# cornell-zhang/HiSparse

Hardware: AMD Instinct MI355X
Metric: SpMV GBPS (8 B per non-zero per SpMV, sw/benchmark.cpp:312-346) (higher is better)
Workload: dtype u32 (Q8.24 fixed point, u64 row sums)

## Files before the change

### hisparse_amd/csrc/spmv_device.h

```cpp
#ifndef HISPARSE_SPMV_DEVICE_H_
#define HISPARSE_SPMV_DEVICE_H_

#include <hip/hip_runtime.h>

#include <type_traits>

#include "stream_tiles.h"

namespace hisparse {
namespace dev {
namespace {

__device__ __forceinline__ uint32_t q8_24_mul(uint32_t a, uint32_t b) {
    const uint64_t wide = static_cast<uint64_t>(a) * b + 0x800000ull;
    uint32_t hi = static_cast<uint32_t>(wide >> 32);
    const uint32_t lo = static_cast<uint32_t>(wide);
    asm("" : "+v"(hi));
    const uint32_t r = __builtin_amdgcn_alignbit(hi, lo, 24);
    return (hi >> 24) ? 0xffffffffu : r;
}

typedef const __attribute__((address_space(4))) Unit* UnitTable;
typedef const __attribute__((address_space(4))) Block* BlockTable;

template <bool kFloat>
struct Rows;
template <>
struct Rows<false> {
    using acc_t = unsigned long long;
    using prod_t = unsigned long long;
    static __device__ __forceinline__ prod_t product(uint32_t mat, uint32_t vec) { return q8_24_mul(mat, vec); }
    static __device__ __forceinline__ void add(acc_t* ys, uint32_t row, prod_t p) { atomicAdd(ys + row, p); }
    static __device__ __forceinline__ uint32_t finish(acc_t s) { return s > 0xffffffffull ? 0xffffffffu : static_cast<uint32_t>(s); }
    using sum_t = unsigned long long;
    static __device__ __forceinline__ sum_t widen(prod_t p) { return p; }
    static __device__ __forceinline__ void add_sum(acc_t* ys, uint32_t row, sum_t v) { atomicAdd(ys + row, v); }
    using lane_t = unsigned long long;
    static __device__ __forceinline__ void add_lane(acc_t* ys, uint32_t row, lane_t v) { atomicAdd(ys + row, v); }
};
template <>
struct Rows<true> {
    using acc_t = double;
    using prod_t = float;
    static __device__ __forceinline__ prod_t product(uint32_t mat, uint32_t vec) { return __uint_as_float(mat) * __uint_as_float(vec); }
    static __device__ __forceinline__ void add(acc_t* ys, uint32_t row, prod_t p) { atomicAdd(ys + row, static_cast<double>(p)); }
    static __device__ __forceinline__ uint32_t finish(acc_t s) { return __float_as_uint(static_cast<float>(s)); }
    using sum_t = double;
    static __device__ __forceinline__ sum_t widen(prod_t p) { return static_cast<double>(p); }
    static __device__ __forceinline__ void add_sum(acc_t* ys, uint32_t row, sum_t v) { atomicAdd(ys + row, v); }
    using lane_t = float;
    static __device__ __forceinline__ void add_lane(acc_t* ys, uint32_t row, lane_t v) { atomicAdd(ys + row, static_cast<double>(v)); }
};

template <typename T>
__device__ __forceinline__ T wave_sum(T v) {
#pragma unroll
    for (int m = 32; m >= 1; m >>= 1) v += __shfl_xor(v, m, kWaveLanes);
    return v;
}

template <int kCtrl, int kRowMask>
__device__ __forceinline__ uint32_t dpp_from(uint32_t v) {
    return static_cast<uint32_t>(__builtin_amdgcn_update_dpp(0, static_cast<int>(v), kCtrl, kRowMask, 0xf, false));
}
template <int kCtrl, int kRowMask>
__device__ __forceinline__ unsigned long long dpp_from(unsigned long long v) {
    const uint32_t lo = dpp_from<kCtrl, kRowMask>(static_cast<uint32_t>(v)), hi = dpp_from<kCtrl, kRowMask>(static_cast<uint32_t>(v >> 32));
    return static_cast<unsigned long long>(hi) << 32 | lo;
}
template <int kCtrl, int kRowMask>
__device__ __forceinline__ double dpp_from(double v) {
    return __longlong_as_double(static_cast<long long>(dpp_from<kCtrl, kRowMask>(static_cast<unsigned long long>(__double_as_longlong(v)))));
}
template <typename T>
__device__ __forceinline__ T wave_inclusive_scan(T v);
template <typename T>
__device__ __forceinline__ T wave_total_in_lane63(T v) { return wave_inclusive_scan(v); }
template <typename T>
__device__ __forceinline__ T wave_inclusive_scan(T v) {
    v += dpp_from<0x111, 0xf>(v);
    v += dpp_from<0x112, 0xf>(v);
    v += dpp_from<0x114, 0xf>(v);
    v += dpp_from<0x118, 0xf>(v);
    v += dpp_from<0x142, 0xa>(v);
    v += dpp_from<0x143, 0xc>(v);
    return v;
}

template <int kCtrl, int kRowMask, typename T>
__device__ __forceinline__ void segmented_step(T& v, uint32_t row) {
    const uint32_t from_row = static_cast<uint32_t>(__builtin_amdgcn_update_dpp(-1, static_cast<int>(row), kCtrl, kRowMask, 0xf, false));
    const T arriving = dpp_from<kCtrl, kRowMask>(v);
    if (from_row == row) v += arriving;
}
template <typename T>
__device__ __forceinline__ T segmented_run_sums(T v, uint32_t row, bool& is_last) {
    segmented_step<0x111, 0xf>(v, row);
    segmented_step<0x112, 0xf>(v, row);
    segmented_step<0x114, 0xf>(v, row);
    segmented_step<0x118, 0xf>(v, row);
    segmented_step<0x142, 0xa>(v, row);
    segmented_step<0x143, 0xc>(v, row);
    const uint32_t next_row = static_cast<uint32_t>(__builtin_amdgcn_update_dpp(-1, static_cast<int>(row), 0x130, 0xf, 0xf, false));
    is_last = next_row != row;
    return v;
}


struct CarriedCombine {
    const uint32_t* partial = nullptr;
    uint32_t* y = nullptr;
    uint32_t num_rows = 0;
    uint32_t slices = 0;
};

// ... 48 lines not shown
```

### hisparse_amd/csrc/spmv_kernels.hip

```cpp
#include <hip/hip_runtime.h>

#include <cstdio>
#include <cstdlib>
#include <utility>
#include <vector>

#include "spmv_kernels.h"
#include "spmv_device.h"

namespace hisparse {
namespace dev {

namespace {

constexpr int kThreads = kWaveLanes * kWavesPerWorkgroup;
constexpr int kLightThreads = 256;
#ifndef HS_LIGHT_BATCH
#define HS_LIGHT_BATCH 4
#endif
constexpr int kLightBatch = HS_LIGHT_BATCH;
constexpr uint32_t kBufBytes = kSubTileCols * 4u;

template <int kIters, int kStride>
__device__ __forceinline__ void fill_x(uint32_t* dst, const uint32_t* __restrict__ x, uint32_t col0, uint32_t ncols, uint32_t t) {
// ... 20 lines not shown
}
template <int kFills>
__device__ __forceinline__ void dma_wait() {
    asm volatile("s_waitcnt vmcnt(%0)" ::"n"(kFills * kDmaPerFill) : "memory");
}

#ifndef HS_ROWBLOCK_STREAM_POLICY
#define HS_ROWBLOCK_STREAM_POLICY "nt"
#endif
#ifndef HS_ROWBLOCK_RESIDENT_POLICY
#define HS_ROWBLOCK_RESIDENT_POLICY "sc1"
#endif
#define HS_BY_POLICY(kRes, STATEMENT)                                 \
    do {                                                              \
        if constexpr (kRes) { STATEMENT(HS_ROWBLOCK_RESIDENT_POLICY); } \
        else { STATEMENT(HS_ROWBLOCK_STREAM_POLICY); }                \
    } while (0)
#define HS_RING_AGPRS "a0", "a1", "a2", "a3", "a4", "a5", "a6", "a7", "a8", "a9", "a10", "a11", "a12", "a13", "a14", "a15", "a16", "a17", \
                      "a18", "a19", "a20", "a21", "a22", "a23", "a24", "a25", "a26", "a27", "a28", "a29", "a30", "a31"
constexpr int kMaxDepth = 16;
constexpr int kOwner24Depth = 3;

constexpr int ring_format(int kRing) { return (kRing & 8) ? 4 : (kRing & 3); }
constexpr bool ring_is_delta(int kRing) { return ring_format(kRing) == 1 || ring_format(kRing) == 4; }
template <int kFmt, bool kRes>
struct RingT;
template <int kRing>
using Ring = RingT<ring_format(kRing), (kRing & 4) != 0>;
template <bool kRes>
struct RingT<0, kRes> {
    static constexpr uint32_t kLaneBytes = 8;
    template <int K>
    static __device__ __forceinline__ void issue(const uint8_t* base, uint32_t byte_off, uint32_t lane_off) {
#define HS_ISSUE(P) asm volatile("s_nop 4\n\tglobal_load_dwordx2 a[%0:%1], %2, %3 " P ::"n"(2 * K), "n"(2 * K + 1), "v"(byte_off + lane_off), "s"(base) : "memory", HS_RING_AGPRS)
        HS_BY_POLICY(kRes, HS_ISSUE);
#undef HS_ISSUE
    }
    template <int K, int kDepth>
    static __device__ __forceinline__ void take(uint32_t& value, uint32_t& where) {
        asm volatile("s_waitcnt vmcnt(%4)\n\tv_accvgpr_read_b32 %0, a[%2]\n\tv_accvgpr_read_b32 %1, a[%3]"
                     : "=v"(value), "=v"(where) : "n"(2 * K), "n"(2 * K + 1), "n"(kDepth - 1) : "memory");
    }
    template <int K, int kDepth>
    static __device__ __forceinline__ void take2(uint32_t& value0, uint32_t& where0, uint32_t& value1, uint32_t& where1) {
        asm volatile("s_waitcnt vmcnt(%8)\n\tv_accvgpr_read_b32 %0, a[%4]\n\tv_accvgpr_read_b32 %1, a[%5]\n\tv_accvgpr_read_b32 %2, a[%6]\n\t"
                     "v_accvgpr_read_b32 %3, a[%7]"
                     : "=v"(value0), "=v"(where0), "=v"(value1), "=v"(where1)
                     : "n"(2 * K), "n"(2 * K + 1), "n"(2 * K + 2), "n"(2 * K + 3), "n"(kDepth - 2) : "memory");
    }
};
template <bool kRes>
struct RingT<1, kRes> {
    static constexpr uint32_t kLaneBytes = 8;
    template <int K>
    static __device__ __forceinline__ void issue(const uint8_t* base, uint32_t byte_off, uint32_t lane_off) {
        static_assert(2 * K + 1 < kMaxDepth && K + kMaxDepth < 2 * kMaxDepth, "values in a0..a15, gap words in a16..a23: ring depth <= 8");
#define HS_ISSUE(P)                                                                                                                                         \
    asm volatile("s_nop 4\n\tglobal_load_dwordx2 a[%0:%1], %3, %5 " P "\n\tglobal_load_dword a[%2], %4, %5 offset:512 " P ::"n"(2 * K), "n"(2 * K + 1),     \
                 "n"(K + kMaxDepth), "v"(byte_off + lane_off), "v"(byte_off + lane_off / 2), "s"(base)                                                     \
                 : "memory", HS_RING_AGPRS)
        HS_BY_POLICY(kRes, HS_ISSUE);
#undef HS_ISSUE
    }
    template <int K, int kDepth>
    static __device__ __forceinline__ void take_record(uint32_t& value_a, uint32_t& value_b, uint32_t& gaps) {
        asm volatile("s_waitcnt vmcnt(%6)\n\tv_accvgpr_read_b32 %0, a[%3]\n\tv_accvgpr_read_b32 %1, a[%4]\n\tv_accvgpr_read_b32 %2, a[%5]"
                     : "=v"(value_a), "=v"(value_b), "=v"(gaps) : "n"(2 * K), "n"(2 * K + 1), "n"(K + kMaxDepth), "n"(2 * (kDepth - 1)) : "memory");
    }
};
template <bool kRes>
struct RingT<4, kRes> {
    static constexpr uint32_t kLaneBytes = 8;
    template <int K>
    static __device__ __forceinline__ void issue(const uint8_t* base, uint32_t byte_off, uint32_t lane_off) {
        static_assert(2 * K + 1 < kMaxDepth && K + kMaxDepth < 2 * kMaxDepth, "dwordx2 in a0..a15, gap B in a16..a23: ring depth <= 8");
#define HS_ISSUE(P)                                                                                                                                         \
    asm volatile("s_nop 4\n\tglobal_load_dwordx2 a[%0:%1], %3, %5 " P "\n\tglobal_load_ushort a[%2], %4, %5 offset:512 " P ::"n"(2 * K), "n"(2 * K + 1),    \
                 "n"(K + kMaxDepth), "v"(byte_off + lane_off), "v"(byte_off + lane_off / 4), "s"(base)                                                     \
                 : "memory", HS_RING_AGPRS)
        HS_BY_POLICY(kRes, HS_ISSUE);
#undef HS_ISSUE
    }
    template <int K, int kDepth>
    static __device__ __forceinline__ void take_record(uint32_t& field_a, uint32_t& field_b, uint32_t& gaps) {
        uint32_t lo, hi, gap_b;
        asm volatile("s_waitcnt vmcnt(%6)\n\tv_accvgpr_read_b32 %0, a[%3]\n\tv_accvgpr_read_b32 %1, a[%4]\n\tv_accvgpr_read_b32 %2, a[%5]"
                     : "=v"(lo), "=v"(hi), "=v"(gap_b) : "n"(2 * K), "n"(2 * K + 1), "n"(K + kMaxDepth), "n"(2 * (kDepth - 1)) : "memory");
        field_a = lo & 0xffffffu;
        field_b = __builtin_amdgcn_alignbit(hi, lo, 24) & 0xffffffu;
        gaps = (hi >> 16) | (gap_b << 16);
    }
};
template <bool kRes>
struct RingT<2, kRes> {
    static constexpr uint32_t kLaneBytes = 4;
    template <int K>
    static __device__ __forceinline__ void issue(const uint8_t* base, uint32_t byte_off, uint32_t lane_off) {
#define HS_ISSUE(P)                                                                                                                       \
    asm volatile("s_nop 4\n\tglobal_load_dword a[%0], %2, %4 " P "\n\tglobal_load_dword a[%1], %3, %4 offset:256 " P ::"n"(K),           \
                 "n"(K + kMaxDepth), "v"(byte_off + lane_off), "v"(byte_off + lane_off - lane_off / 4), "s"(base)                        \
                 : "memory", HS_RING_AGPRS)
        HS_BY_POLICY(kRes, HS_ISSUE);
#undef HS_ISSUE
    }
    template <int K, int kDepth>
    static __device__ __forceinline__ void take(uint32_t& value, uint32_t& where) {
        asm volatile("s_waitcnt vmcnt(%4)\n\tv_accvgpr_read_b32 %0, a[%2]\n\tv_accvgpr_read_b32 %1, a[%3]"
                     : "=v"(value), "=v"(where) : "n"(K), "n"(K + kMaxDepth), "n"(2 * (kDepth - 1)) : "memory");
        where &= 0xffffffu;
    }
    template <int K, int kDepth>
    static __device__ __forceinline__ void take2(uint32_t& value0, uint32_t& where0, uint32_t& value1, uint32_t& where1) {
        asm volatile("s_waitcnt vmcnt(%8)\n\tv_accvgpr_read_b32 %0, a[%4]\n\tv_accvgpr_read_b32 %1, a[%5]\n\tv_accvgpr_read_b32 %2, a[%6]\n\t"
                     "v_accvgpr_read_b32 %3, a[%7]"
                     : "=v"(value0), "=v"(where0), "=v"(value1), "=v"(where1)
                     : "n"(K), "n"(K + kMaxDepth), "n"(K + 1), "n"(K + 1 + kMaxDepth), "n"(2 * (kDepth - 2)) : "memory");
        where0 &= 0xffffffu;
        where1 &= 0xffffffu;
    }
};
template <bool kRes>
struct RingT<3, kRes> {
    template <int K>
    static __device__ __forceinline__ void issue(const uint8_t* base, uint32_t byte_off, uint32_t lane16, uint32_t lane12) {
        static_assert(K < 4 && 16 + 4 * K + 2 < 2 * kMaxDepth, "a0..a15: values of four records, a16..a30: their position words");
#define HS_ISSUE(P)                                                                                                                                          \
    asm volatile("s_nop 4\n\tglobal_load_dwordx4 a[%0:%1], %4, %6 " P "\n\tglobal_load_dwordx3 a[%2:%3], %5, %6 offset:1024 " P ::"n"(4 * K), "n"(4 * K + 3), \
                 "n"(16 + 4 * K), "n"(16 + 4 * K + 2), "v"(byte_off + lane16), "v"(byte_off + lane12), "s"(base)                                            \
                 : "memory", HS_RING_AGPRS)
        HS_BY_POLICY(kRes, HS_ISSUE);
#undef HS_ISSUE
    }
    template <int K, int kDepth>
    static __device__ __forceinline__ void take(uint32_t (&v)[4], uint32_t (&w)[3]) {
        asm volatile("s_waitcnt vmcnt(%14)\n\tv_accvgpr_read_b32 %0, a[%7]\n\tv_accvgpr_read_b32 %1, a[%8]\n\tv_accvgpr_read_b32 %2, a[%9]\n\t"
                     "v_accvgpr_read_b32 %3, a[%10]\n\tv_accvgpr_read_b32 %4, a[%11]\n\tv_accvgpr_read_b32 %5, a[%12]\n\tv_accvgpr_read_b32 %6, a[%13]"
                     : "=v"(v[0]), "=v"(v[1]), "=v"(v[2]), "=v"(v[3]), "=v"(w[0]), "=v"(w[1]), "=v"(w[2])
                     : "n"(4 * K), "n"(4 * K + 1), "n"(4 * K + 2), "n"(4 * K + 3), "n"(16 + 4 * K), "n"(16 + 4 * K + 1), "n"(16 + 4 * K + 2), "n"(2 * (kDepth - 1))
                     : "memory");
    }
};
__device__ __forceinline__ const uint8_t* scalar_pointer(const uint8_t* p) {
    const uint64_t a = reinterpret_cast<uint64_t>(p);
    const uint32_t hi = __builtin_amdgcn_readfirstlane(static_cast<uint32_t>(a >> 32));
    const uint32_t lo = __builtin_amdgcn_readfirstlane(static_cast<uint32_t>(a));
    return reinterpret_cast<const uint8_t*>((static_cast<uint64_t>(hi) << 32) | lo);
}

__device__ __forceinline__ void lds_barrier() {
    __builtin_amdgcn_fence(__ATOMIC_RELEASE, "workgroup", "local");
    __builtin_amdgcn_s_barrier();
    __builtin_amdgcn_fence(__ATOMIC_ACQUIRE, "workgroup", "local");
}

template <bool kFloat> struct OwnerSum { using type = float; };
template <> struct OwnerSum<false> { using type = uint32_t; };
template <bool kFloat>
struct Consumer {
    using acc_t = typename Rows<kFloat>::acc_t;
    using prod_t = typename Rows<kFloat>::prod_t;
    static constexpr uint32_t kNoRow = 0xffffffffu;
    const uint8_t* stream;
    UnitTable unit;
    uint32_t U, wave, lane, lane_off, ring, nrows, last;
    const uint32_t* xs;
    acc_t* ys;
    uint32_t u = 0, slot = 0, end = 0, base = 0;
    uint32_t next_end = 0;
    const uint32_t* xb;
    uint32_t pos = 0;
    uint32_t value_shift = 0;
    bool head = true;
    uint32_t run_row = kNoRow;
    typename Rows<kFloat>::sum_t run_sum = 0;
    uint32_t lane_row = 0;
    typename Rows<kFloat>::lane_t lane_sum = 0;
    typename OwnerSum<kFloat>::type own_sum = 0;
    uint32_t spare = 0;
    uint32_t row_base = 0;
    uint32_t lane_off12 = 0;
    uint64_t t_flush = 0, t_barrier = 0;
};

__device__ uint64_t* g_owner_profile = nullptr;
__device__ uint64_t* g_rowblock_timeline = nullptr;
constexpr uint32_t kTimelineBlocks = 4, kTimelineStamps = 8;
template <int kAblate>
__device__ __forceinline__ void timeline_stamp(uint32_t k, uint32_t wave, uint32_t lane, uint32_t i) {
    if (!(kAblate & 512)) return;
    if (lane != 0 || (wave != 0 && wave != kConsumerWaves) || k >= kTimelineBlocks || !g_rowblock_timeline) return;
    const uint64_t t = __builtin_amdgcn_s_memrealtime();
    g_rowblock_timeline[((static_cast<size_t>(blockIdx.x) * kTimelineBlocks + k) * 2 + (wave ? 1 : 0)) * kTimelineStamps + i] = t;
}

template <bool kFloat, int kRing, int kAblate, int kDepth, bool kDense, int K>
__device__ __forceinline__ bool consume_step(Consumer<kFloat>& c) {
    using R = Rows<kFloat>;
    constexpr bool kDelta = ring_is_delta(kRing), kPacked = ring_format(kRing) == 4, k24 = ring_format(kRing) == 2;
    constexpr uint32_t kStride = kPacked ? kRecordBytes24 : kDelta ? kRecordBytes : k24 ? kWaveStrideBytes24 : kWaveStrideBytes;
    constexpr uint32_t kColMask = k24 ? kSubTileCols - 1u : 0xffffu, kRowShift = k24 ? kOwnerColBits : 16u;
    const uint32_t s = c.base + K;
    while (s == c.end) {
        if (!kDelta && kDense && c.u + 1 == c.U && c.run_row != Consumer<kFloat>::kNoRow) {
            const typename R::sum_t sum = wave_sum(c.run_sum);
            if (c.lane == 0) R::add_sum(c.ys, c.run_row, sum);
            c.run_row = Consumer<kFloat>::kNoRow;
        }
        if (kDelta && kDense) {
            R::add_lane(c.ys, c.lane_row, c.lane_sum);
            c.lane_row = c.nrows;
            c.lane_sum = 0;
        }
        if (!(kAblate & 8)) lds_barrier();
        if (++c.u == c.U) return false;
        c.end = c.next_end;
        c.next_end = c.unit[min(c.u + 1, c.U - 1)].end_step[c.wave];
        c.slot = c.slot + 1 == c.ring ? 0 : c.slot + 1;
        c.xb = c.xs + c.slot * kSubTileCols;
        c.head = true;
    }
    uint32_t mat, aux;
    if constexpr (kDelta) {
        uint32_t value_a, value_b, gaps;
        Ring<kRing>::template take_record<K, kDepth>(value_a, value_b, gaps);
        auto slot = [&](uint32_t value, uint32_t gap) {
            c.pos += gap;
            uint32_t row = c.pos / kSubTileCols;
            const uint32_t col = c.pos % kSubTileCols;
            if (kAblate & 1) {
                asm volatile("" ::"v"(row), "v"(value));
                return;
            }
            const uint32_t xv = (kAblate & 2) ? col : c.xb[col];
            typename R::prod_t prod = R::product(value, xv);
            if (kFloat) {
                if (gap == kBridgeGap) prod = 0;
                row = min(row, c.nrows);
            }
            if (kDense) {
                if (row != c.lane_row) {
                    R::add_lane(c.ys, c.lane_row, c.lane_sum);
                    c.lane_row = row;
                    c.lane_sum = 0;
                }
                c.lane_sum += prod;
            } else {
                R::add(c.ys, row, prod);
            }
        };
        if (c.head) {
            c.pos = kPacked ? (value_a | (gaps << 24)) : value_a;
            c.head = false;
        } else {
            slot(kPacked ? value_a << c.value_shift : value_a, gaps & 0xffffu);
        }
        slot(kPacked ? value_b << c.value_shift : value_b, gaps >> 16);
    } else {
        Ring<kRing>::template take<K, kDepth>(mat, aux);
        const uint32_t xv = (kAblate & 2) ? aux : c.xb[aux & kColMask];
        if (kAblate & 1) {
            asm volatile("" ::"v"(xv), "v"(mat));
        } else {
            const typename R::prod_t prod = R::product(mat, xv);
            const uint32_t row = aux >> kRowShift;
            if (kDense) {
                const uint32_t row0 = __builtin_amdgcn_readfirstlane(row);
                const bool uniform = __ballot(row == row0) == ~0ull;
                if (uniform && row0 == c.run_row) {
                    c.run_sum += R::widen(prod);
                } else {
                    if (c.run_row != Consumer<kFloat>::kNoRow) {
                        const typename R::sum_t sum = wave_sum(c.run_sum);
                        if (c.lane == 0) R::add_sum(c.ys, c.run_row, sum);
                    }
                    if (uniform) { c.run_row = row0; c.run_sum = R::widen(prod); }
                    else { c.run_row = Consumer<kFloat>::kNoRow; c.run_sum = 0; R::add(c.ys, row, prod); }
                }
            } else {
                R::add(c.ys, row, prod);
            }
        }
    }
    Ring<kRing>::template issue<K>(c.stream, min(s + kDepth, c.last) * kStride, c.lane_off);
    return true;
}

template <bool kFloat>
struct OwnerOps;
template <>
struct OwnerOps<true> {
    using val_t = float;
    static __device__ __forceinline__ val_t product(uint32_t mat, uint32_t xv) { return __uint_as_float(mat) * __uint_as_float(xv); }
    static __device__ __forceinline__ val_t add(val_t a, val_t b) { return a + b; }
};
template <>
struct OwnerOps<false> {
    using val_t = uint32_t;
    static __device__ __forceinline__ val_t product(uint32_t mat, uint32_t xv) { return q8_24_mul(mat, xv); }
    static __device__ __forceinline__ val_t add(val_t a, val_t b) { return __builtin_elementwise_add_sat(a, b); }
};
template <bool kFloat>
__device__ __forceinline__ void owner_flush(typename OwnerOps<kFloat>::val_t* ys32, uint32_t row, typename OwnerOps<kFloat>::val_t sum) {
    ys32[row] = OwnerOps<kFloat>::add(ys32[row], sum);
}
template <bool kFloat>
__device__ __forceinline__ void owner_end_of_unit(Consumer<kFloat>& c) {
    using Ops = OwnerOps<kFloat>;
    using val_t = typename Ops::val_t;
    val_t* ys32 = reinterpret_cast<val_t*>(c.ys);
    const uint32_t row = c.lane_row;
    val_t sum = c.own_sum;
    const bool live = row != c.spare;
    const uint32_t above = __shfl_down(row, 1, kWaveLanes);
    const bool same_above = live && c.lane + 1 < kWaveLanes && above == row;
    if (__ballot(same_above) == 0) {
        if (live) owner_flush<kFloat>(ys32, row, sum);
    } else {
#pragma unroll
        for (uint32_t d = 1; d < kWaveLanes; d <<= 1) {
            const val_t s2 = __shfl_down(sum, d, kWaveLanes);
            const uint32_t r2 = __shfl_down(row, d, kWaveLanes);
            if (c.lane + d < kWaveLanes && r2 == row) sum = Ops::add(sum, s2);
        }
        const uint32_t below = __shfl_up(row, 1, kWaveLanes);
        if (live && (c.lane == 0 || below != row)) owner_flush<kFloat>(ys32, row, sum);
    }
    c.lane_row = c.spare;
    c.own_sum = 0;
}

template <int kRing, int kAblate, int kDepth, int K>
__device__ __forceinline__ bool consume_step_owner(Consumer<true>& c) {
    constexpr uint32_t kStep = kChunkBytes;
    static_assert(kRing == 0, "8-byte OWNER chunks");
    const uint32_t s = c.base + K;
    while (s == c.end) {
        if (kAblate & 256) {
            const uint64_t t0 = __builtin_readcyclecounter();
            owner_end_of_unit(c);
// ... 210 lines not shown

template <bool kFloat, int kRing, int kDepth, bool kOwner = false>
__device__ __forceinline__ void consumer_begin(Consumer<kFloat>& c, const uint8_t* stream, UnitTable unit, uint32_t U, uint32_t wave,
                                               uint32_t lane, const uint32_t* xs, uint32_t ring, typename Rows<kFloat>::acc_t* ys, uint32_t nrows,
                                               uint32_t total, uint32_t first_end) {
    static_assert(kDepth <= kMaxDepth, "the ring lives in a0..a31");
    constexpr bool kDelta = ring_is_delta(kRing), kPacked = ring_format(kRing) == 4, k24 = ring_format(kRing) == 2;
    constexpr uint32_t kStride = kPacked ? kRecordBytes24 : kDelta ? kRecordBytes : kOwner ? kChunkBytes : k24 ? kWaveStrideBytes24 : kWaveStrideBytes;
    c.stream = scalar_pointer(stream);
    c.unit = unit; c.U = U; c.wave = wave; c.lane = lane; c.ring = ring; c.nrows = nrows;
    c.lane_off = lane * Ring<kRing>::kLaneBytes;
    c.last = total ? total - 1 : 0;
    c.xs = xs; c.xb = xs; c.ys = ys;
    c.end = first_end;
    c.next_end = U > 1 ? unit[1].end_step[wave] : first_end;
    c.lane_row = kOwner ? nrows + wave : nrows;
    c.spare = nrows + wave;
    prime_ring<kRing>(c.stream, c.last, kStride, c.lane_off, std::make_integer_sequence<int, kDepth>());
}

template <bool kFloat, int kRing, int kAblate, int kDepth, bool kDense, bool kOwner = false>
__device__ __forceinline__ void consumer_run(Consumer<kFloat>& c) {
    __builtin_amdgcn_s_waitcnt(0x0f70);
    if (kAblate & 64) { c.u = c.U - 1; c.end = c.last + 1; }
    const uint64_t t_begin = (kOwner && (kAblate & 256)) ? __builtin_readcyclecounter() : 0;
    for (;; c.base += kDepth) {
        if constexpr (kOwner) {
            if (!consume_round_owner<kRing, kAblate, kDepth>(c, std::make_integer_sequence<int, kDepth>())) break;
        } else {
            if (!consume_round<kFloat, kRing, kAblate, kDepth, kDense>(c, std::make_integer_sequence<int, kDepth>())) break;
        }
    }
    asm volatile("s_waitcnt vmcnt(0)" ::: "memory", HS_RING_AGPRS);
    if (kOwner && (kAblate & 256) && c.lane == 0 && g_owner_profile) {
        uint64_t* p = g_owner_profile + (static_cast<size_t>(blockIdx.x) * kWavesPerWorkgroup + c.wave) * 8;
        p[0] += __builtin_readcyclecounter() - t_begin;
        p[1] += c.t_flush;
        p[2] += c.t_barrier;
        p[3] += c.U;
        p[4] += c.last + 1;
    }
}

template <bool kFloat, int kRing, int kAblate, int kDepth, bool kOwner = false>
__device__ __forceinline__ void rowblock_workgroup(const uint8_t* __restrict__ image, const Block* __restrict__ blocks,
                                                   const Unit* __restrict__ units, const uint32_t* __restrict__ x,
                                                   uint32_t* __restrict__ out, int32_t row_part_filter, uint32_t ring,
                                                   uint32_t x_base, const uint32_t* __restrict__ part_heads, const CarriedCombine& carry) {
    using acc_t = typename Rows<kFloat>::acc_t;
    extern __shared__ __attribute__((aligned(16))) uint8_t lds[];
    acc_t* ys = reinterpret_cast<acc_t*>(lds);
    uint32_t* xs = reinterpret_cast<uint32_t*>(lds + x_base);
    const uint32_t tid = threadIdx.x;
    const uint32_t lane = tid & (kWaveLanes - 1);
    const uint32_t wave = __builtin_amdgcn_readfirstlane(tid / kWaveLanes);
    const bool loader = wave >= kConsumerWaves;
    uint32_t wg = blockIdx.x;
    if ((gridDim.x & 7u) == 0) wg = (blockIdx.x & 7u) * (gridDim.x >> 3) + (blockIdx.x >> 3);

    uint32_t bi = wg;
    if (row_part_filter >= 0) {
        bi = ((const __attribute__((address_space(4))) uint32_t*)part_heads)[static_cast<uint32_t>(row_part_filter) * gridDim.x + wg];
        if (bi == kNoBlock) return;
    }
    bool first_block = true;
    uint32_t block_no = 0;
    for (uint32_t next = 0;; bi = next, ++block_no) {
        const BlockTable blk = (BlockTable)(blocks + bi);
        next = (row_part_filter >= 0 && blk->next_part > static_cast<uint32_t>(row_part_filter)) ? 0u : blk->next;
        const uint32_t nrows = blk->nrows, out0 = blk->out_offset;
        const UnitTable unit = (UnitTable)(units + blk->unit_begin);
        const uint32_t U = blk->unit_end - blk->unit_begin;

        if (!first_block) __syncthreads();
        first_block = false;
        timeline_stamp<kAblate>(block_no, wave, lane, 0);
        Consumer<kFloat> c;
        if (!loader && U > 0) {
            if constexpr (kRing == 3)
                consumer_begin_owner24<kFloat, kDepth>(c, image + blk->wave_offset[wave], unit, U, wave, lane, xs, ring, ys, nrows, blk->total_steps[wave], blk->first_end[wave]);
            else
                consumer_begin<kFloat, kRing, kDepth, kOwner>(c, image + blk->wave_offset[wave], unit, U, wave, lane, xs, ring, ys, nrows, blk->total_steps[wave],
                                                               blk->first_end[wave]);
            if constexpr (ring_format(kRing) == 4) c.value_shift = blk->value_shift;
        }
        if (carry.partial && block_no == 0) carried_combine<kFloat, kThreads>(carry, blockIdx.x, gridDim.x, tid);
        if (kOwner) {
            if (!(kAblate & 16)) for (uint32_t i = tid; i < nrows + kConsumerWaves; i += kThreads) reinterpret_cast<float*>(ys)[i] = 0.0f;
        } else
        if (!(kAblate & 16)) for (uint32_t i = tid; i <= nrows; i += kThreads) ys[i] = 0;
        if (U > 0 && !(kAblate & 16)) fill_x<kSubTileCols / 4 / kThreads, kThreads>(xs, x, blk->first_col0, blk->first_ncols, tid);
        __syncthreads();
        timeline_stamp<kAblate>(block_no, wave, lane, 1);

        if (U > 0) {
            if (loader) {
                const uint32_t lw = wave - kConsumerWaves;
                __builtin_amdgcn_s_setprio(3);
                uint32_t fill_slot = 1 == ring ? 0 : 1;
                uint32_t col0_next = U > 1 ? unit[1].col0 : 0, ncols_next = U > 1 ? unit[1].ncols : 8;
                uint32_t col0_after = U > 2 ? unit[2].col0 : col0_next, ncols_after = U > 2 ? unit[2].ncols : ncols_next;
                auto refill = [&](uint32_t v) {
                    const uint32_t col0 = col0_next, ncols = ncols_next;
                    if (kOwner) {
                        col0_next = col0_after;
                        ncols_next = ncols_after;
                        const uint32_t ahead = min(v + 2, U - 1);
                        col0_after = unit[ahead].col0;
                        ncols_after = unit[ahead].ncols;
                    } else {
                        const uint32_t ahead = min(v + 1, U - 1);
                        col0_next = unit[ahead].col0;
                        ncols_next = unit[ahead].ncols;
                    }
                    if (!(kAblate & 4)) dma_fill_x(xs + fill_slot * kSubTileCols, x, col0, ncols, lw, lane);
                    fill_slot = fill_slot + 1 == ring ? 0 : fill_slot + 1;
                };
                uint32_t issued = 1;
                while (issued < U && issued < ring - 1) refill(issued++);
                uint64_t t_wait = 0, t_bar = 0, t_issue = 0;
                const uint64_t t_begin = (kOwner && (kAblate & 256)) ? __builtin_readcyclecounter() : 0;
                for (uint32_t u = 0; u < U; ++u) {
                    const uint64_t ti = (kOwner && (kAblate & 256)) ? __builtin_readcyclecounter() : 0;
                    if (issued < U) refill(issued++);
                    if (kOwner && (kAblate & 256)) t_issue += __builtin_readcyclecounter() - ti;
                    const uint32_t younger = issued - min(issued, u + 2);
                    const uint64_t t0 = (kOwner && (kAblate & 256)) ? __builtin_readcyclecounter() : 0;
                    if (younger >= 2) dma_wait<2>(); else if (younger == 1) dma_wait<1>(); else dma_wait<0>();
                    const uint64_t t1 = (kOwner && (kAblate & 256)) ? __builtin_readcyclecounter() : 0;
                    if (!(kAblate & 8)) __builtin_amdgcn_s_barrier();
                    if (kOwner && (kAblate & 256)) { const uint64_t t2 = __builtin_readcyclecounter(); t_wait += t1 - t0; t_bar += t2 - t1; }
                }
                if (kOwner && (kAblate & 256) && lane == 0 && g_owner_profile) {
                    uint64_t* p = g_owner_profile + (static_cast<size_t>(blockIdx.x) * kWavesPerWorkgroup + wave) * 8;
                    p[0] += __builtin_readcyclecounter() - t_begin;
                    p[1] += t_wait;
                    p[2] += t_bar;
                    p[3] += U;
                    p[4] += t_issue;
                }
            } else {
                if constexpr (kRing == 3) consumer_run_owner24<kFloat, kAblate, kDepth>(c);
                else if constexpr (kOwner) consumer_run<kFloat, kRing, kAblate, kDepth, false, true>(c);
                else if (blk->flags & kBlockDenseRows) consumer_run<kFloat, kRing, kAblate, kDepth, true>(c);
                else consumer_run<kFloat, kRing, kAblate, kDepth, false>(c);
            }
        }
        timeline_stamp<kAblate>(block_no, wave, lane, 2);
        if (kOwner) {
            if (!loader) {
                const float flushed = reinterpret_cast<volatile float*>(ys)[nrows + wave];
                asm volatile("" ::"v"(flushed));
            }
            __syncthreads();
            timeline_stamp<kAblate>(block_no, wave, lane, 3);
            if (!(kAblate & 32)) for (uint32_t i = tid; i < nrows; i += kThreads) out[out0 + i] = reinterpret_cast<uint32_t*>(ys)[i];
            timeline_stamp<kAblate>(block_no, wave, lane, 4);
            if (!next) break;
            continue;
        }
        if constexpr (ring_format(kRing) == 4) {
            const uint32_t n_out = blk->outlier_count;
            if (!loader && n_out) {
                const Outlier* list = reinterpret_cast<const Outlier*>(image + ((static_cast<uint64_t>(blk->outlier_hi) << 32) | blk->outlier_lo));
                for (uint32_t i = tid; i < n_out; i += kConsumerWaves * kWaveLanes) {
                    const Outlier o = list[i];
                    Rows<kFloat>::add(ys, o.row, Rows<kFloat>::product(o.value, x[o.col]));
                }
            }
        }
        if (!loader) {
            const acc_t flushed = atomicAdd(ys + nrows, static_cast<acc_t>(0));
            asm volatile("" ::"v"(flushed));
        }
        __syncthreads();
        timeline_stamp<kAblate>(block_no, wave, lane, 3);
        if (!(kAblate & 32)) for (uint32_t i = tid; i < nrows; i += kThreads) out[out0 + i] = Rows<kFloat>::finish(ys[i]);
        timeline_stamp<kAblate>(block_no, wave, lane, 4);
        if (!next) break;
    }
}

template <bool kFloat, int kRing, int kAblate, int kDepth, bool kOwner = false>
__global__ __launch_bounds__(kThreads) void spmv_rowblock_kernel(const uint8_t* __restrict__ image, const Block* __restrict__ blocks,
                                                                  const Unit* __restrict__ units, const uint32_t* __restrict__ x,
                                                                  uint32_t* __restrict__ out, int32_t row_part_filter, uint32_t ring,
                                                                  uint32_t x_base, const uint32_t* __restrict__ part_heads, CarriedCombine carry) {
    static_assert(!(kRing & 8), "DELTA with 24-bit value fields is spmv_rowblock_kernel_delta24");
    rowblock_workgroup<kFloat, kRing, kAblate, kDepth, kOwner>(image, blocks, units, x, out, row_part_filter, ring, x_base, part_heads, carry);
}

template <bool kRes, int kAblate>
__global__ __launch_bounds__(kThreads) void spmv_rowblock_kernel_delta24(const uint8_t* __restrict__ image, const Block* __restrict__ blocks,
                                                                 const Unit* __restrict__ units, const uint32_t* __restrict__ x,
                                                                 uint32_t* __restrict__ out, int32_t row_part_filter, uint32_t ring,
                                                                 uint32_t x_base, const uint32_t* __restrict__ part_heads, CarriedCombine carry) {
    rowblock_workgroup<false, kRes ? 12 : 8, kAblate, 8>(image, blocks, units, x, out, row_part_filter, ring, x_base, part_heads, carry);
}

template <bool kFloat>
__device__ __forceinline__ uint32_t feedback_word(uint32_t y, uint32_t scale, uint32_t shift) {
    if (kFloat) {
        const float p = __uint_as_float(scale) * __uint_as_float(y);
        return __float_as_uint(p + __uint_as_float(shift));
    }
    const uint64_t s = static_cast<uint64_t>(q8_24_mul(scale, y)) + shift;
    return s > 0xffffffffull ? 0xffffffffu : static_cast<uint32_t>(s);
}

template <bool kFloat, int kSlices>
__global__ __launch_bounds__(256) void combine_slices_kernel(const uint32_t* __restrict__ partial, uint32_t* __restrict__ y,
                                                             uint32_t num_rows, uint32_t row_lo, uint32_t row_hi,
                                                             uint32_t* __restrict__ x_fb, uint32_t n_fb, uint32_t scale, uint32_t shift) {
    const uint32_t r = row_lo + (blockIdx.x * blockDim.x + threadIdx.x) * 4u;
    if (r >= row_hi) return;
    uint4 p[kSlices];
#pragma unroll
    for (int k = 0; k < kSlices; ++k) p[k] = *reinterpret_cast<const uint4*>(partial + static_cast<size_t>(k) * num_rows + r);
    uint32_t word[4];
    if (kFloat) {
        float s[4] = {0.0f, 0.0f, 0.0f, 0.0f};
#pragma unroll
        for (int k = 0; k < kSlices; ++k) {
            s[0] += __uint_as_float(p[k].x); s[1] += __uint_as_float(p[k].y); s[2] += __uint_as_float(p[k].z); s[3] += __uint_as_float(p[k].w);
        }
        for (int j = 0; j < 4; ++j) word[j] = __float_as_uint(s[j]);
    } else {
        uint64_t s[4] = {0, 0, 0, 0};
#pragma unroll
        for (int k = 0; k < kSlices; ++k) {
            s[0] += p[k].x; s[1] += p[k].y; s[2] += p[k].z; s[3] += p[k].w;
        }
        for (int j = 0; j < 4; ++j) word[j] = s[j] > 0xffffffffull ? 0xffffffffu : static_cast<uint32_t>(s[j]);
    }
    *reinterpret_cast<uint4*>(y + r) = make_uint4(word[0], word[1], word[2], word[3]);
    if (x_fb && r < n_fb)
        *reinterpret_cast<uint4*>(x_fb + r) = make_uint4(feedback_word<kFloat>(word[0], scale, shift), feedback_word<kFloat>(word[1], scale, shift),
                                                         feedback_word<kFloat>(word[2], scale, shift), feedback_word<kFloat>(word[3], scale, shift));
}

template <bool kFloat>
__global__ __launch_bounds__(256) void feedback_kernel(const uint32_t* __restrict__ y, uint32_t* __restrict__ x, uint32_t n, uint32_t scale,
                                                       uint32_t shift) {
    const uint32_t i = blockIdx.x * blockDim.x + threadIdx.x;
    if (i < n) x[i] = feedback_word<kFloat>(y[i], scale, shift);
}

struct PushTargets { uint32_t* dst[kMaxPushTargets]; };
__global__ __launch_bounds__(256) void push_result_kernel(const uint32_t* __restrict__ y, PushTargets t, uint32_t n_dst, uint32_t words) {
    const uint32_t i = (blockIdx.x * blockDim.x + threadIdx.x) * 4u;
// ... 104 lines not shown
            } else {
                R::add_sum(ys, lane_row, lane_sum);
            }
        }
        const acc_t flushed = atomicAdd(ys + nrows, static_cast<acc_t>(0));
        asm volatile("" ::"v"(flushed));
        __syncthreads();
        if (!(kAblate & 32)) for (uint32_t i = tid; i < nrows; i += kLightThreads) out[out0 + i] = R::finish(ys[i]);
        if (!next) break;
    }
}

template <bool kFloat, int kRing, int kAblate, int kDepth, bool kOwner = false>
hipError_t configure_one(uint32_t lds_bytes) {
    return hipFuncSetAttribute(reinterpret_cast<const void*>(&spmv_rowblock_kernel<kFloat, kRing, kAblate, kDepth, kOwner>),
                               hipFuncAttributeMaxDynamicSharedMemorySize, static_cast<int>(lds_bytes));
}

int env_int(const char* name, int dflt) {
    const char* e = std::getenv(name);
    return e ? std::atoi(e) : dflt;
}

}

bool profiling_depth_given() {
#ifdef HISPARSE_PROFILING
    return std::getenv("HISPARSE_DEPTH") != nullptr;
#else
    return false;
#endif
}
bool profiling_switches(int& ablate, int& depth) {
#ifdef HISPARSE_PROFILING
    ablate = env_int("HISPARSE_ABLATE", 0);
    depth = env_int("HISPARSE_DEPTH", 8);
    return true;
#else
    ablate = 0;
    depth = 8;
    return profiling_switch_error() == nullptr;
#endif
}
const char* profiling_switch_error() {
#ifdef HISPARSE_PROFILING
    return nullptr;
#else
    if (env_int("HISPARSE_ABLATE", 0) != 0)
        return "HISPARSE_ABLATE is set: the ablation builds (wrong results by design) live in libhisparse_hip_prof.so (make HISPARSE_PROFILING=1, "
               "HISPARSE_HIP_LIB=...); this library will not launch with it in the environment";
    if (env_int("HISPARSE_DEPTH", 8) != 8)
        return "HISPARSE_DEPTH is set: prefetch-depth experiments live in libhisparse_hip_prof.so (make HISPARSE_PROFILING=1); this library will "
               "not launch with it in the environment";
    return nullptr;
#endif
}

uint32_t spmv_light_lds_bytes(uint32_t max_block_rows) { return ((max_block_rows + 1) * kAccumulatorBytes + 15u) & ~15u; }
uint32_t spmv_lds_bytes(uint32_t max_block_rows, uint32_t ring_buffers, uint32_t format) {
    const uint32_t acc = (format == kFormatOwner || format == kFormatOwner24) ? (max_block_rows + kConsumerWaves) * kOwnerAccumulatorBytes : (max_block_rows + 1) * kAccumulatorBytes;
    return ((acc + 15u) & ~15u) + ring_buffers * kBufBytes;
}

#ifdef HISPARSE_PROFILING
#define HS_FOR_EACH_OWNER24_ABLATION(X) X(0) X(1) X(4) X(5) X(8) X(12) X(13) X(512)
#define HS_FOR_EACH_LIGHT_VARIANT(X) X(0) X(1) X(2) X(3) X(32) X(35)
#define HS_FOR_EACH_OWNER24_DEPTH(X) X(2) X(3) X(4)
#define HS_FOR_EACH_OWNER24_FIXED(X) X(0) X(512)
#define HS_FOR_EACH_OWNER_VARIANT(X) X(0) X(1) X(2) X(3) X(4) X(7) X(8) X(11) X(12) X(15) X(127) X(256)
#else
#define HS_FOR_EACH_OWNER24_ABLATION(X) X(0)
#define HS_FOR_EACH_LIGHT_VARIANT(X) X(0)
#define HS_FOR_EACH_OWNER24_DEPTH(X) X(3)
#define HS_FOR_EACH_OWNER24_FIXED(X) X(0)
#define HS_FOR_EACH_OWNER_VARIANT(X) X(0)
#endif

#define HS_FOR_EACH_PRODUCT_VARIANT(X)                                                                           \
    X(true, 0, 0, 8) X(true, 1, 0, 8) X(false, 0, 0, 8) X(false, 1, 0, 8) X(true, 2, 0, 8) X(false, 2, 0, 8)      \
    X(true, 4, 0, 8) X(true, 5, 0, 8) X(false, 4, 0, 8) X(false, 5, 0, 8)
#ifndef HISPARSE_PROFILING
#define HS_FOR_EACH_DELTA24_VARIANT(X) X(false, 0) X(true, 0)
#else
#define HS_FOR_EACH_DELTA24_VARIANT(X) X(false, 0) X(true, 0) X(false, 1) X(false, 2) X(false, 3)
#endif
#ifndef HISPARSE_PROFILING
#define HS_FOR_EACH_VARIANT(X) HS_FOR_EACH_PRODUCT_VARIANT(X)
#else
#define HS_FOR_EACH_VARIANT(X)                                                                                   \
    HS_FOR_EACH_PRODUCT_VARIANT(X)                                                                               \
    X(false, false, 0, 16) X(false, false, 3, 8) X(false, true, 3, 8)                       \
    X(false, false, 4, 8) X(false, true, 4, 8) X(false, false, 8, 8) X(false, true, 8, 8) X(false, false, 15, 8) X(false, true, 15, 8) X(false, false, 31, 8) X(false, true, 31, 8)                     \
    X(false, false, 47, 8) X(false, true, 47, 8) X(false, false, 79, 8) X(false, true, 79, 8)                     \
    X(false, false, 127, 8) X(false, true, 127, 8)                                                                 \
    X(true, false, 3, 8) X(true, false, 4, 8) X(true, false, 8, 8) X(true, false, 15, 8) X(true, false, 127, 8) \
    X(false, false, 512, 8) X(false, true, 512, 8) X(true, false, 512, 8) X(true, true, 512, 8)
#endif

hipError_t configure_spmv_kernels(uint32_t lds_bytes) {
    hipError_t e;
#define X(F, T, A, D) if ((e = configure_one<F, T, A, D>(lds_bytes)) != hipSuccess) return e;
    HS_FOR_EACH_VARIANT(X)
#undef X
#define X(R, A)                                                                                                                               \
    if ((e = hipFuncSetAttribute(reinterpret_cast<const void*>(&spmv_rowblock_kernel_delta24<R, A>), hipFuncAttributeMaxDynamicSharedMemorySize, \
                                 static_cast<int>(lds_bytes))) != hipSuccess)                                                                \
        return e;
    HS_FOR_EACH_DELTA24_VARIANT(X)
#undef X
#define X(A) if ((e = configure_one<true, false, A, 8, true>(lds_bytes)) != hipSuccess) return e;
    HS_FOR_EACH_OWNER_VARIANT(X)
#undef X
#define X(D) if (D != 3 && (e = configure_one<true, 3, 0, D, true>(lds_bytes)) != hipSuccess) return e;
    HS_FOR_EACH_OWNER24_DEPTH(X)
#undef X
#define X(A) if ((e = configure_one<true, 3, A, 3, true>(lds_bytes)) != hipSuccess) return e;
    HS_FOR_EACH_OWNER24_ABLATION(X)
#undef X
#define X(A) if ((e = configure_one<false, 3, A, 3, true>(lds_bytes)) != hipSuccess) return e;
    HS_FOR_EACH_OWNER24_FIXED(X)
#undef X
    if ((e = configure_sweep_kernels(lds_bytes)) != hipSuccess) return e;
    return configure_bitmap_kernels(lds_bytes);
}

hipError_t launch_spmv(bool is_float, const SpmvLaunch& a, hipStream_t stream) {
    if (a.num_workgroups == 0) return hipSuccess;
    if (a.format == kFormatBitmap) return launch_spmv_bitmap(is_float, a, stream);
    if (a.format == kFormatSweep) return launch_spmv_sweep(is_float, a, stream);
    if (a.light) {
        if (a.format != kFormatPairs) return hipErrorInvalidValue;
        int ablate = 0, depth_unused = 8;
        if (!profiling_switches(ablate, depth_unused)) return hipErrorInvalidValue;
        const dim3 grid(a.num_workgroups), block(kLightThreads);
#define X(A)                                                                                                                                  \
    if (ablate == A) {                                                                                                                        \
        if (is_float) hipLaunchKernelGGL((spmv_light_kernel<true, A>), grid, block, a.lds_bytes, stream, a.image, a.blocks, a.units, a.x, a.out, a.row_part_filter, a.part_heads); \
        else hipLaunchKernelGGL((spmv_light_kernel<false, A>), grid, block, a.lds_bytes, stream, a.image, a.blocks, a.units, a.x, a.out, a.row_part_filter, a.part_heads);       \
        return hipGetLastError();                                                                                                             \
    }
        HS_FOR_EACH_LIGHT_VARIANT(X)
#undef X
        return hipErrorInvalidValue;
    }
    int ring = a.format == kFormatDelta ? 1 : a.format == kFormatPairs24 ? 2 : 0;
    const bool delta24 = a.format == kFormatDelta && a.value_bits == 24;
    if (delta24 && is_float) return hipErrorInvalidValue;
    const dim3 grid(a.num_workgroups), block(kThreads);
    const uint32_t x_base = a.lds_bytes - a.ring_buffers * kBufBytes;
    const CarriedCombine carry = carried(a);
    int ablate = 0, depth = 8;
    if (!profiling_switches(ablate, depth)) return hipErrorInvalidValue;
    if (a.stream_resident && ring < 2 && ablate == 0 && depth == 8 && (a.format == kFormatPairs || a.format == kFormatDelta)) ring |= 4;
    bool launched = false;
    struct TimelineDump {
        hipStream_t stream; uint32_t workgroups; bool on;
        ~TimelineDump() {
            const char* path = std::getenv("HISPARSE_TIMELINE_OUT");
            if (!on || !path || !buffer()) return;
            (void)hipStreamSynchronize(stream);
            std::vector<uint64_t> host(size_t(workgroups) * kTimelineBlocks * 2 * kTimelineStamps);
            (void)hipMemcpy(host.data(), buffer(), host.size() * sizeof(uint64_t), hipMemcpyDeviceToHost);
            if (FILE* f = std::fopen(path, "wb")) { std::fwrite(host.data(), sizeof(uint64_t), host.size(), f); std::fclose(f); }
        }
        static uint64_t*& buffer() {
            static uint64_t* b[16] = {};
            int dev = 0;
            (void)hipGetDevice(&dev);
            return b[dev >= 0 && dev < 16 ? dev : 0];
        }
    } timeline_dump{stream, a.num_workgroups, ablate == 512 && a.num_workgroups <= 4096};
    if (timeline_dump.on) {
        const size_t bytes = size_t(4096) * kTimelineBlocks * 2 * kTimelineStamps * sizeof(uint64_t);
        if (!TimelineDump::buffer() && hipMalloc(reinterpret_cast<void**>(&TimelineDump::buffer()), bytes) == hipSuccess)
            (void)hipMemcpyToSymbol(HIP_SYMBOL(g_rowblock_timeline), &TimelineDump::buffer(), sizeof(uint64_t*));
        if (TimelineDump::buffer()) (void)hipMemsetAsync(TimelineDump::buffer(), 0, bytes, stream);
    }
    if (a.format == kFormatOwner24) {
        const int records = profiling_depth_given() ? depth : kOwner24Depth;
        if (!is_float) {
            if (records != 3) return hipErrorInvalidValue;
#define X(A)                                                                                                                       \
    if (ablate == A) {                                                                                                             \
        hipLaunchKernelGGL((spmv_rowblock_kernel<false, 3, A, 3, true>), grid, block, a.lds_bytes, stream, a.image, a.blocks, a.units, a.x, a.out, \
                           a.row_part_filter, a.ring_buffers, x_base, a.part_heads, carry);                                               \
        return hipGetLastError();                                                                                                  \
    }
            HS_FOR_EACH_OWNER24_FIXED(X)
#undef X
            return hipErrorInvalidValue;
        }
#define X(A)                                                                                                                       \
    if (ablate == A && records == 3) {                                                                                             \
        hipLaunchKernelGGL((spmv_rowblock_kernel<true, 3, A, 3, true>), grid, block, a.lds_bytes, stream, a.image, a.blocks, a.units, a.x, a.out, \
                           a.row_part_filter, a.ring_buffers, x_base, a.part_heads, carry);                                               \
        return hipGetLastError();                                                                                                  \
    }
        HS_FOR_EACH_OWNER24_ABLATION(X)
#undef X
        if (ablate != 0) return hipErrorInvalidValue;
#define X(D)                                                                                                                       \
    if (records == D) {                                                                                                            \
        hipLaunchKernelGGL((spmv_rowblock_kernel<true, 3, 0, D, true>), grid, block, a.lds_bytes, stream, a.image, a.blocks, a.units, a.x, a.out, \
                           a.row_part_filter, a.ring_buffers, x_base, a.part_heads, carry);                                               \
        return hipGetLastError();                                                                                                  \
    }
        HS_FOR_EACH_OWNER24_DEPTH(X)
#undef X
        return hipErrorInvalidValue;
    }
    if (a.format == kFormatOwner) {
        if (!is_float) return hipErrorInvalidValue;
        static uint64_t* profile = nullptr;
        if (ablate == 256 && !profile) {
            (void)hipMalloc(reinterpret_cast<void**>(&profile), size_t(4096) * kWavesPerWorkgroup * 8 * sizeof(uint64_t));
            (void)hipMemset(profile, 0, size_t(4096) * kWavesPerWorkgroup * 8 * sizeof(uint64_t));
            (void)hipMemcpyToSymbol(HIP_SYMBOL(g_owner_profile), &profile, sizeof(profile));
        }
#define X(A)                                                                                                                      \
    if (!launched && ablate == A) {                                                                                               \
        hipLaunchKernelGGL((spmv_rowblock_kernel<true, false, A, 8, true>), grid, block, a.lds_bytes, stream, a.image, a.blocks,  \
                           a.units, a.x, a.out, a.row_part_filter, a.ring_buffers, x_base, a.part_heads, carry);                        \
        launched = true;                                                                                                          \
    }
        if (depth == 8) {
        HS_FOR_EACH_OWNER_VARIANT(X)
        }
#undef X
        if (ablate == 256 && profile && a.num_workgroups <= 4096) {
            if (const char* path = std::getenv("HISPARSE_TIMELINE_OUT")) {
                (void)hipStreamSynchronize(stream);
                std::vector<uint64_t> host(size_t(a.num_workgroups) * kWavesPerWorkgroup * 8);
                (void)hipMemcpy(host.data(), profile, host.size() * sizeof(uint64_t), hipMemcpyDeviceToHost);
                if (FILE* f = std::fopen(path, "wb")) {
                    std::fwrite(host.data(), sizeof(uint64_t), host.size(), f);
                    std::fclose(f);
// ... 67 lines not shown
```

Baseline: 7334.

## Track packed delta24 positions as flat offsets and decode fields with byte perms

```diff
diff --git a/hisparse_amd/csrc/spmv_device.h b/hisparse_amd/csrc/spmv_device.h
--- a/hisparse_amd/csrc/spmv_device.h
+++ b/hisparse_amd/csrc/spmv_device.h
@@ -20,6 +20,10 @@
     return (hi >> 24) ? 0xffffffffu : r;
 }
 
+__device__ __forceinline__ uint32_t q8_24_mul_below_one(uint32_t value8, uint32_t b) {
+    return static_cast<uint32_t>((static_cast<uint64_t>(value8) * b + 0x80000000ull) >> 32);
+}
+
 typedef const __attribute__((address_space(4))) Unit* UnitTable;
 typedef const __attribute__((address_space(4))) Block* BlockTable;
 
@@ -31,6 +35,9 @@
     using prod_t = unsigned long long;
     static __device__ __forceinline__ prod_t product(uint32_t mat, uint32_t vec) { return q8_24_mul(mat, vec); }
     static __device__ __forceinline__ void add(acc_t* ys, uint32_t row, prod_t p) { atomicAdd(ys + row, p); }
+    static __device__ __forceinline__ void add_at(uint32_t byte_offset, prod_t p) {
+        __hip_atomic_fetch_add((__attribute__((address_space(3))) acc_t*)byte_offset, p, __ATOMIC_RELAXED, __HIP_MEMORY_SCOPE_AGENT);
+    }
     static __device__ __forceinline__ uint32_t finish(acc_t s) { return s > 0xffffffffull ? 0xffffffffu : static_cast<uint32_t>(s); }
     using sum_t = unsigned long long;
     static __device__ __forceinline__ sum_t widen(prod_t p) { return p; }
diff --git a/hisparse_amd/csrc/spmv_kernels.hip b/hisparse_amd/csrc/spmv_kernels.hip
--- a/hisparse_amd/csrc/spmv_kernels.hip
+++ b/hisparse_amd/csrc/spmv_kernels.hip
@@ -126,14 +126,14 @@
 #undef HS_ISSUE
     }
     template <int K, int kDepth>
-    static __device__ __forceinline__ void take_record(uint32_t& field_a, uint32_t& field_b, uint32_t& gaps) {
-        uint32_t lo, hi, gap_b;
+    static __device__ __forceinline__ void take_record(uint32_t& lo, uint32_t& hi, uint32_t& gap_b) {
         asm volatile("s_waitcnt vmcnt(%6)\n\tv_accvgpr_read_b32 %0, a[%3]\n\tv_accvgpr_read_b32 %1, a[%4]\n\tv_accvgpr_read_b32 %2, a[%5]"
                      : "=v"(lo), "=v"(hi), "=v"(gap_b) : "n"(2 * K), "n"(2 * K + 1), "n"(K + kMaxDepth), "n"(2 * (kDepth - 1)) : "memory");
-        field_a = lo & 0xffffffu;
-        field_b = __builtin_amdgcn_alignbit(hi, lo, 24) & 0xffffffu;
-        gaps = (hi >> 16) | (gap_b << 16);
-    }
+    }
+    static constexpr uint32_t kFieldA = 0x0c020100u, kFieldB = 0x0c050403u;
+    static constexpr uint32_t kFieldA8 = 0x0201000cu, kFieldB8 = 0x0504030cu;
+    static constexpr uint32_t kGapA = 0x0c0c0706u, kHeadPos = 0x06020100u, kNone = 0x0c0c0c0cu;
+    static __device__ __forceinline__ uint32_t bytes(uint32_t hi, uint32_t lo, uint32_t selector) { return __builtin_amdgcn_perm(hi, lo, selector); }
 };
 template <bool kRes>
 struct RingT<2, kRes> {
@@ -251,8 +251,13 @@
             c.run_row = Consumer<kFloat>::kNoRow;
         }
         if (kDelta && kDense) {
-            R::add_lane(c.ys, c.lane_row, c.lane_sum);
-            c.lane_row = c.nrows;
+            if constexpr (kPacked) {
+                R::add_at(c.lane_row, c.lane_sum);
+                c.lane_row = c.nrows * static_cast<uint32_t>(sizeof(typename R::acc_t));
+            } else {
+                R::add_lane(c.ys, c.lane_row, c.lane_sum);
+                c.lane_row = c.nrows;
+            }
             c.lane_sum = 0;
         }
         if (!(kAblate & 8)) lds_barrier();
@@ -262,9 +267,51 @@
         c.slot = c.slot + 1 == c.ring ? 0 : c.slot + 1;
         c.xb = c.xs + c.slot * kSubTileCols;
         c.head = true;
+        if constexpr (kPacked) c.pos = 0;
     }
     uint32_t mat, aux;
-    if constexpr (kDelta) {
+    if constexpr (kPacked) {
+        using P = Ring<kRing>;
+        constexpr uint32_t kAccBytes = static_cast<uint32_t>(sizeof(typename R::acc_t));
+        static_assert(!kFloat && kAccBytes == 8 && kSubTileCols == 8192, "fixed point only; row offset = (pos >> 13) * 8");
+        uint32_t lo, hi, gap_b;
+        P::template take_record<K, kDepth>(lo, hi, gap_b);
+        const bool head = c.head;
+        c.head = false;
+        const uint32_t pos_a = c.pos + P::bytes(hi, lo, head ? P::kHeadPos : P::kGapA), pos_b = pos_a + gap_b;
+        c.pos = pos_b;
+        const uint32_t sel_a = head ? P::kNone : P::kFieldA, sel_a8 = head ? P::kNone : P::kFieldA8;
+        auto gather = [&](uint32_t pos) { return (kAblate & 2) ? pos % kSubTileCols : c.xb[pos % kSubTileCols]; };
+        auto row_of = [](uint32_t pos) { return (pos / kSubTileCols) * kAccBytes; };
+        auto record = [&](auto below_one) {
+            auto product = [&](uint32_t sel, uint32_t sel8, uint32_t xv) -> typename R::prod_t {
+                if constexpr (decltype(below_one)::value) return q8_24_mul_below_one(P::bytes(hi, lo, sel8), xv);
+                else return R::product(P::bytes(hi, lo, sel) << c.value_shift, xv);
+            };
+            if (kAblate & 1) {
+                asm volatile("" ::"v"(row_of(pos_a)), "v"(row_of(pos_b)), "v"(P::bytes(hi, lo, sel_a8)), "v"(P::bytes(hi, lo, P::kFieldB8)));
+            } else {
+                auto slot = [&](uint32_t pos, uint32_t sel, uint32_t sel8) {
+                    const typename R::prod_t prod = product(sel, sel8, gather(pos));
+                    if (kDense) {
+                        const uint32_t row = row_of(pos);
+                        if (row != c.lane_row) {
+                            R::add_at(c.lane_row, c.lane_sum);
+                            c.lane_row = row;
+                            c.lane_sum = 0;
+                        }
+                        c.lane_sum += prod;
+                    } else {
+                        R::add_at(row_of(pos), prod);
+                    }
+                };
+                slot(pos_a, sel_a, sel_a8);
+                slot(pos_b, P::kFieldB, P::kFieldB8);
+            }
+        };
+        if (__builtin_expect(c.value_shift == 0, 1)) record(std::true_type());
+        else record(std::false_type());
+    } else if constexpr (kDelta) {
         uint32_t value_a, value_b, gaps;
         Ring<kRing>::template take_record<K, kDepth>(value_a, value_b, gaps);
         auto slot = [&](uint32_t value, uint32_t gap) {
@@ -293,12 +340,12 @@
             }
         };
         if (c.head) {
-            c.pos = kPacked ? (value_a | (gaps << 24)) : value_a;
+            c.pos = value_a;
             c.head = false;
         } else {
-            slot(kPacked ? value_a << c.value_shift : value_a, gaps & 0xffffu);
-        }
-        slot(kPacked ? value_b << c.value_shift : value_b, gaps >> 16);
+            slot(value_a, gaps & 0xffffu);
+        }
+        slot(value_b, gaps >> 16);
     } else {
         Ring<kRing>::template take<K, kDepth>(mat, aux);
         const uint32_t xv = (kAblate & 2) ? aux : c.xb[aux & kColMask];
@@ -675,7 +722,10 @@
             else
                 consumer_begin<kFloat, kRing, kDepth, kOwner>(c, image + blk->wave_offset[wave], unit, U, wave, lane, xs, ring, ys, nrows, blk->total_steps[wave],
                                                                blk->first_end[wave]);
-            if constexpr (ring_format(kRing) == 4) c.value_shift = blk->value_shift;
+            if constexpr (ring_format(kRing) == 4) {
+                c.value_shift = blk->value_shift;
+                c.lane_row = nrows * static_cast<uint32_t>(sizeof(acc_t));
+            }
         }
         if (carry.partial && block_no == 0) carried_combine<kFloat, kThreads>(carry, blockIdx.x, gridDim.x, tid);
         if (kOwner) {
@@ -758,7 +808,7 @@
                 const Outlier* list = reinterpret_cast<const Outlier*>(image + ((static_cast<uint64_t>(blk->outlier_hi) << 32) | blk->outlier_lo));
                 for (uint32_t i = tid; i < n_out; i += kConsumerWaves * kWaveLanes) {
                     const Outlier o = list[i];
-                    Rows<kFloat>::add(ys, o.row, Rows<kFloat>::product(o.value, x[o.col]));
+                    Rows<kFloat>::add_at(o.row * static_cast<uint32_t>(sizeof(acc_t)), Rows<kFloat>::product(o.value, x[o.col]));
                 }
             }
         }
@@ -1029,7 +1079,7 @@
 #ifndef HISPARSE_PROFILING
 #define HS_FOR_EACH_DELTA24_VARIANT(X) X(false, 0) X(true, 0)
 #else
-#define HS_FOR_EACH_DELTA24_VARIANT(X) X(false, 0) X(true, 0) X(false, 1) X(false, 2) X(false, 3)
+#define HS_FOR_EACH_DELTA24_VARIANT(X) X(false, 0) X(true, 0) X(false, 1) X(false, 2) X(false, 3) X(true, 1) X(true, 2) X(true, 3)
 #endif
 #ifndef HISPARSE_PROFILING
 #define HS_FOR_EACH_VARIANT(X) HS_FOR_EACH_PRODUCT_VARIANT(X)
@@ -1098,7 +1148,7 @@
     const CarriedCombine carry = carried(a);
     int ablate = 0, depth = 8;
     if (!profiling_switches(ablate, depth)) return hipErrorInvalidValue;
-    if (a.stream_resident && ring < 2 && ablate == 0 && depth == 8 && (a.format == kFormatPairs || a.format == kFormatDelta)) ring |= 4;
+    if (a.stream_resident && ring < 2 && (ablate == 0 || (delta24 && ablate <= 3)) && depth == 8 && (a.format == kFormatPairs || a.format == kFormatDelta)) ring |= 4;
     bool launched = false;
     struct TimelineDump {
         hipStream_t stream; uint32_t workgroups; bool on;
```

New measurement: 7423 (median of 6 runs). +1.2%, better.
